# yeeus/GCI

Measured on AMD Instinct MI355X. Metric: aligned Gbases/s through filter+depth pipeline (CHM13, 40x HiFi), higher is better.
Workload: dtype int32

## Files before the change

### gci_amd/csrc/api_ctx.hip

```cpp
#include "gci_ctx.hpp"
#include <stdlib.h>
#include <vector>

int gci_fail(gci_ctx* c, hipError_t e, const char* what)
{
    if (c) c->err = std::string(what) + ": " + hipGetErrorString(e);
    return GCI_E_HIP;
}

int gci_ensure(gci_ctx* ctx, DevBuf& b, size_t bytes)
{
    if (bytes <= b.cap) return GCI_OK;
    if (b.p) { HIPCHK(hipStreamSynchronize(ctx->stream)); HIPCHK(gci_dfree(b.p)); b.p = nullptr; b.cap = 0; }
    size_t want = bytes + bytes / 4 + 256;
    HIPCHK(gci_dmalloc(ctx->device, &b.p, want));
    b.cap = want;
    return GCI_OK;
}

int gci_upload_small(gci_ctx* ctx, void* d_dst, const void* h_src, size_t bytes)
{
    HIPCHK(hipStreamSynchronize(ctx->stream));
    if (bytes > ctx->h_pinned_cap) {
        if (ctx->h_pinned) HIPCHK(hipHostFree(ctx->h_pinned));
// ... 18 lines not shown
    ctx->device = device;
    { const char* fd = getenv("GCI_FORCE_DENSE"); if (fd && fd[0] == '1') ctx->sparse_max = -1; }
    { const char* m = getenv("GCI_JOIN"); ctx->join_mode = m && m[0] == 'c' ? 1 : m && m[0] == 'p' ? 2 : 0; }
    { const char* g = getenv("GCI_PAGES_GRID"); const long n = g ? atol(g) : 0; ctx->pg_grid_cap = n > 0 && n < (1 << 20) ? (uint32_t)n : 0u; }
    hipError_t e = hipSetDevice(device);
    if (e != hipSuccess) { delete ctx; return GCI_E_HIP; }
    if (!own_stream) { ctx->stream = (hipStream_t)stream; }
    else {
        e = hipStreamCreateWithFlags(&ctx->stream, hipStreamNonBlocking);
        if (e != hipSuccess) { delete ctx; return GCI_E_HIP; }
        ctx->own_stream = true;
    }
    {
        uint32_t lut[TEXT_LUT];
        gci_text_lut_host(lut);
        if (gci_dmalloc(device, &ctx->text_lut.p, sizeof lut) != hipSuccess ||
            hipMemcpy(ctx->text_lut.p, lut, sizeof lut, hipMemcpyHostToDevice) != hipSuccess) {
            gci_ctx_destroy(ctx);
            return GCI_E_HIP;
        }
        ctx->text_lut.cap = sizeof lut;
    }
    *out = ctx;
    return GCI_OK;
}

extern "C" int gci_ctx_destroy(gci_ctx* ctx)
{
    if (!ctx) return GCI_OK;
    (void)hipSetDevice(ctx->device);
    (void)hipStreamSynchronize(ctx->stream);
    DevBuf* bufs[] = {&ctx->d_len, &ctx->d_off, &ctx->d_tile_first, &ctx->tile_cd, &ctx->tile_carry, &ctx->dense_flag, &ctx->dense_list, &ctx->evp_items, &ctx->evp_hist, &ctx->evp_blk, &ctx->d_tile_valid,
                      &ctx->evt_off, &ctx->events, &ctx->blk_a, &ctx->blk_b, &ctx->tile_sum, &ctx->tile_u32,
                      &ctx->tile_u64, &ctx->blk_u64, &ctx->join_table, &ctx->join_last, &ctx->join_hq, &ctx->part_a, &ctx->part_b, &ctx->part_hist, &ctx->part_blk, &ctx->conflict_table, &ctx->win,
                      &ctx->win_tile_first, &ctx->text_lut, &ctx->long_items, &ctx->pg_scan, &ctx->pg_first, &ctx->pg_list, &ctx->route_tab, &ctx->deflate_nruns, &ctx->deflate_runs, &ctx->deflate_tab, &ctx->dgz_tiles, &ctx->build_nruns, &ctx->build_runs, &ctx->join_bucket, &ctx->tail_gaps, &ctx->tail_sums, &ctx->class_sums, &ctx->crc_tabs, &ctx->inflate_sym, &ctx->inflate_nsym, &ctx->inflate_wstatus, &ctx->inflate_lists, &ctx->inflate_prof, &ctx->inflate_next, &ctx->inflate_sym2, &ctx->inflate_lists2,
                      &ctx->bg_tile_cnt, &ctx->bg_tile_off, &ctx->bg_blk, &ctx->bg_wtab, &ctx->bg_blk_bytes, &ctx->bg_blk_off, &ctx->bg_blk2, &ctx->hist_chunk_first,
                      &ctx->cover_rec, &ctx->cover_chunk, &ctx->fate_rec, &ctx->fate_chunk};
    for (DevBuf* b : bufs) if (b->p) (void)gci_dfree(b->p);
    for (DevBuf& b : ctx->paf_pool) if (b.p) (void)gci_dfree(b.p);
    if (ctx->h_pinned) (void)hipHostFree(ctx->h_pinned);
    for (auto* v : {&ctx->prof_live, &ctx->prof_free}) for (auto& e : *v) { (void)hipEventDestroy(e.a); (void)hipEventDestroy(e.b); }
    if (ctx->inflate_stream2) { (void)hipStreamSynchronize(ctx->inflate_stream2); (void)hipStreamDestroy(ctx->inflate_stream2); }
    if (ctx->inflate_ev_in) (void)hipEventDestroy(ctx->inflate_ev_in);
    if (ctx->inflate_ev_out) (void)hipEventDestroy(ctx->inflate_ev_out);
    if (ctx->own_stream) (void)hipStreamDestroy(ctx->stream);
    delete ctx;
    return GCI_OK;
}

extern "C" int gci_sync(gci_ctx* ctx)
{
    if (!ctx) return GCI_E_INVALID;
    HIPCHK(hipStreamSynchronize(ctx->stream));
    return GCI_OK;
}

extern "C" const char* gci_strerror(int s)
{
    switch (s) {
    case GCI_OK: return "ok";
    case GCI_E_INVALID: return "invalid argument";
    case GCI_E_HIP: return "HIP runtime error";
    case GCI_E_NO_NM: return "record without NM tag (reference raises KeyError, GCI.py:163)";
    case GCI_E_ZERO_DIV: return "zero denominator (reference raises ZeroDivisionError, GCI.py:165/292)";
    case GCI_E_BAD_NM_TYPE: return "NM tag is not an integer";
    case GCI_E_NO_END: return "record has no CIGAR: reference_end is None";
    case GCI_E_MALFORMED: return "malformed BAM record";
// ... 138 lines not shown
```

### gci_amd/csrc/gci_ctx.hpp

```cpp
#pragma once
#include <hip/hip_runtime.h>
#include <stdint.h>
#include <stdlib.h>
#include <string.h>
#include <string>
#include <vector>

#include "../../include/gci_hip.h"
#include "gci_common.h"
#include "gci_wave.hpp"

#define TILE GCI_TILE
#define TEXT_LUT 1000
#define BLOCK 256
static_assert(TILE == BLOCK * 16, "a tile is 16 elements per thread");

constexpr int GCI_RUN_MAX = 64;
constexpr uint32_t GCI_RUNS_WALK = 0xFFFFFFFFu;

struct DevBuf {
    void* p = nullptr;
    size_t cap = 0;
};

// ... 5 lines not shown
    int32_t n_contigs = 0;
    std::vector<int64_t> len, off;
    std::vector<int64_t> tile_first;
    int64_t total = 0, n_tiles = 0;
    DevBuf d_len, d_off, d_tile_first;
    DevBuf tile_cd;
    DevBuf tile_carry;
    DevBuf evt_off;
    DevBuf d_tile_valid;
    DevBuf dense_flag;
    DevBuf dense_list;
    int32_t sparse_max = 62;
    bool join_dirty = false;
    int join_mode = 0;
    uint32_t k1_parity = 0;
    int cd_state = 0;
    int counted_flank = 0;
    bool count_deferred = false;
    DevBuf evp_items, evp_hist, evp_blk;
    DevBuf events;
    DevBuf blk_a, blk_b;
    DevBuf tile_sum;
    DevBuf tile_u32, tile_u64, blk_u64;
    uint32_t build_max_n = 0;
    int build_flank = 0;
    bool build_pending = false, build_text = false;
    bool build_runs_wanted = false;
    DevBuf build_nruns, build_runs;
    const void* build_runs_track = nullptr;
    bool build_runs_armed = false;
    DevBuf join_table, join_last, join_hq;
    DevBuf join_bucket;
    DevBuf part_a, part_b, part_hist, part_blk;
    DevBuf route_tab;
    DevBuf deflate_nruns, deflate_runs;
    DevBuf deflate_tab;
    bool deflate_tab_ready = false;
    DevBuf dgz_tiles;
    uint32_t dgz_members = 0;
    const void* dgz_key = nullptr;
    bool deflate_from_build = false;
    uint32_t deflate_members = 0;
    const void* deflate_key_depth = nullptr;
    const void* deflate_key_elem = nullptr;
    DevBuf conflict_table;
    uint64_t conflict_slots = 0;
    uint32_t conflict_parity = 0;
    DevBuf text_lut;
    DevBuf long_items;
    DevBuf pg_scan, pg_first;
    uint32_t pg_n_rec = 0, pg_page_bytes = 0, pg_n_pages = 0;
    uint32_t pg_cus = 0;
    uint32_t pg_per_cu = 0, pg_per_cu_page_bytes = 0;
    uint32_t pg_lean_per_cu = 0, pg_lean_page_bytes = 0;
    uint32_t pg_grid_cap = 0;
    DevBuf pg_list;
    uint32_t pg_parity = 0;
    uint64_t pg_blob_off = 0;
    uint64_t pg_blob_bytes = 0;
    std::vector<DevBuf> paf_pool;
    DevBuf crc_tabs;
    bool crc_tabs_ready = false;
    uint32_t inflate_last_n = 0;
    DevBuf inflate_sym, inflate_nsym, inflate_wstatus, inflate_lists, inflate_prof, inflate_next;
    DevBuf inflate_sym2, inflate_lists2;
    int inflate_streams = 1;
// ... 377 lines not shown
```

### gci_amd/csrc/k_join.hip

```cpp
#include "gci_ctx.hpp"
#include <stdlib.h>

struct JoinFiles {
    gci_join_file f[GCI_MAX_JOIN_FILES];
    int n;
};

#define SLOT_EMPTY 0xFFFFFFFFFFFFFFFFull

__device__ __forceinline__ const uint8_t* name_ptr(const gci_join_file& f, uint32_t idx)
{
    return f.d_name_base + f.d_name_off[idx] + f.name_delta;
}

__device__ __forceinline__ bool same_name(const JoinFiles& F, int fa, uint32_t ia, const gci_rec& a,
                                          unsigned long long owner)
{
    const int fb = (int)(owner >> 32);
    const uint32_t ib = (uint32_t)owner;
    const gci_rec& b = F.f[fb].d_recs[ib];
    if (a.name_hash != b.name_hash || a.name_len != b.name_len) return false;
    const uint8_t* pa = name_ptr(F.f[fa], ia);
    const uint8_t* pb = name_ptr(F.f[fb], ib);
    for (uint32_t i = 0; i < a.name_len; i++) if (pa[i] != pb[i]) return false;
// ... 175 lines not shown
    atomicMin(status, (unsigned long long)(unsigned)(-GCI_E_CAPACITY));
}

__device__ __forceinline__ int part_file_of(const PartFiles& P, int n, uint32_t chunk)
{
    int f = 0;
    while (f + 1 < n && chunk >= P.chunk_first[f + 1]) f++;
    return f;
}

__device__ __forceinline__ const uint8_t* entry_name(const JoinFiles& F, const PartEntry& e)
{
    return F.f[(e.meta >> PART_CONTIG_BITS) & 15u].d_name_base + (((uint64_t)e.name_off16 << 4) | (uint64_t)(e.key >> 60));
}

__device__ __forceinline__ void store_entry(PartEntry* __restrict__ dst, const PartEntry& e)
{
    int4* d = reinterpret_cast<int4*>(dst);
    d[0] = make_int4((int)(uint32_t)e.key, (int)(uint32_t)(e.key >> 32), (int)e.idx, (int)e.meta);
    d[1] = make_int4(e.start, e.end, e.qlen, (int)e.name_off16);
}

__device__ __forceinline__ PartEntry load_entry(const PartEntry* __restrict__ src)
{
    const int4* s = reinterpret_cast<const int4*>(src);
    const int4 a = s[0], b = s[1];
    PartEntry e;
    e.key = (unsigned long long)(uint32_t)a.x | ((unsigned long long)(uint32_t)a.y << 32);
    e.idx = (uint32_t)a.z; e.meta = (uint32_t)a.w;
    e.start = b.x; e.end = b.y; e.qlen = b.z; e.name_off16 = (uint32_t)b.w;
    return e;
}

__global__ __launch_bounds__(BLOCK) void k_part1_hist(JoinFiles F, PartFiles P, int shift, uint32_t n_bins, uint32_t n_chunks,
                                                      uint32_t* __restrict__ hist, uint32_t* __restrict__ reset_n_out,
                                                      unsigned long long* __restrict__ status)
{
    __shared__ uint32_t h[256];
    const uint32_t t = threadIdx.x, chunk = blockIdx.x;
    if (chunk == 0 && t == 0) *reset_n_out = 0;
    h[t] = 0;
    __syncthreads();
    const int f = part_file_of(P, F.n, chunk);
    const uint32_t i0 = (chunk - P.chunk_first[f]) * PART_CHUNK, n = F.f[f].n_recs;
    const gci_rec* __restrict__ recs = F.f[f].d_recs;
#pragma unroll 4
    for (int k = 0; k < PART_CHUNK / BLOCK; k++) {
        const uint32_t i = i0 + k * BLOCK + t;
        if (i < n) {
            const gci_rec r = recs[i];
            if (part_takes(r)) atomicAdd(&h[(uint32_t)((r.name_hash & PART_KEY_MASK) >> shift) & (n_bins - 1)], 1u);
            else if (r.flags & GCI_REC_PASS) part_refuse(status);
        }
    }
    __syncthreads();
    if (t < n_bins) hist[(size_t)t * n_chunks + chunk] = h[t];
}

#define SC_TILE 1024
#define SC_PER (SC_TILE / BLOCK)
struct ScatterLds {
    int4 stage[SC_TILE * 2];
    uint32_t tcnt[256], toff[256], gofs[256], cnt[256], base[256];
    uint32_t wtot[BLOCK / 64], total;
    uint8_t sbin[SC_TILE];
};

__device__ __forceinline__ void scatter_tile(ScatterLds& L, const PartEntry (&e)[SC_PER], const int (&d)[SC_PER], uint32_t n_bins,
                                             PartEntry* __restrict__ out, int t)
{
    const int lane = t & 63, wave = t >> 6;
    uint32_t r[SC_PER];
#pragma unroll
    for (int k = 0; k < SC_PER; k++) r[k] = d[k] >= 0 ? atomicAdd(&L.tcnt[d[k]], 1u) : 0u;
    __syncthreads();
    const uint32_t c = (uint32_t)t < n_bins ? L.tcnt[t] : 0u;
    const uint32_t inc = wave_inclusive<uint32_t>(c, lane);
    if (lane == 63) L.wtot[wave] = inc;
    __syncthreads();
    uint32_t pre = inc - c, all = 0;
#pragma unroll
    for (int w = 0; w < BLOCK / 64; w++) { if (w < wave) pre += L.wtot[w]; all += L.wtot[w]; }
    L.toff[t] = pre;
    L.gofs[t] = L.base[t] + L.cnt[t] - pre;
    if (t == 0) L.total = all;
    __syncthreads();
#pragma unroll
    for (int k = 0; k < SC_PER; k++) {
        if (d[k] >= 0) {
            const uint32_t p = L.toff[d[k]] + r[k];
            L.stage[2 * p] = make_int4((int)(uint32_t)e[k].key, (int)(uint32_t)(e[k].key >> 32), (int)e[k].idx, (int)e[k].meta);
            L.stage[2 * p + 1] = make_int4(e[k].start, e[k].end, e[k].qlen, (int)e[k].name_off16);
            L.sbin[p] = (uint8_t)d[k];
        }
    }
    __syncthreads();
    const uint32_t total = L.total;
    for (uint32_t q = t; q < 2 * total; q += BLOCK) {
        const uint32_t p = q >> 1;
        const uint32_t bin = L.sbin[p];
        reinterpret_cast<int4*>(out + (L.gofs[bin] + p))[q & 1] = L.stage[q];
    }
    L.cnt[t] += c;
    L.tcnt[t] = 0;
    __syncthreads();
}

__global__ __launch_bounds__(BLOCK) void k_part1_scatter(JoinFiles F, PartFiles P, int shift, uint32_t n_bins, uint32_t n_chunks,
                                                         const uint32_t* __restrict__ off, PartEntry* __restrict__ out,
                                                         unsigned long long* __restrict__ status)
{
    __shared__ ScatterLds L;
    const uint32_t t = threadIdx.x, chunk = blockIdx.x;
    L.cnt[t] = 0; L.tcnt[t] = 0;
    L.base[t] = t < n_bins ? off[(size_t)t * n_chunks + chunk] : 0u;
    __syncthreads();
    const int f = part_file_of(P, F.n, chunk);
    const uint32_t i0 = (chunk - P.chunk_first[f]) * PART_CHUNK, n = F.f[f].n_recs;
    const gci_rec* __restrict__ recs = F.f[f].d_recs;
    const uint64_t* __restrict__ noff = F.f[f].d_name_off;
    const uint64_t delta = F.f[f].name_delta;
    for (uint32_t tile = 0; tile < PART_CHUNK && i0 + tile < n; tile += SC_TILE) {
        PartEntry e[SC_PER];
        int d[SC_PER];
#pragma unroll
        for (int k = 0; k < SC_PER; k++) {
            const uint32_t i = i0 + tile + k * BLOCK + t;
            d[k] = -1;
            e[k].key = 0; e[k].idx = 0; e[k].meta = 0; e[k].start = e[k].end = e[k].qlen = 0; e[k].name_off16 = 0;
            if (i < n) {
                const gci_rec r = recs[i];
                if (part_takes(r)) {
                    const uint64_t at = noff[i] + delta;
                    if (at >> 36) part_refuse(status);
                    e[k].key = (r.name_hash & PART_KEY_MASK) | ((unsigned long long)r.name_len << 48) | ((unsigned long long)(at & 15ull) << 60);
                    e[k].idx = i;
                    e[k].meta = (uint32_t)r.contig | ((uint32_t)f << PART_CONTIG_BITS) | ((r.flags & GCI_REC_HQ) ? 1u << 30 : 0u) |
                                ((r.flags & GCI_REC_NAME16) ? 1u << 31 : 0u);
                    e[k].start = r.start; e[k].end = r.end; e[k].qlen = r.qlen;
                    e[k].name_off16 = (uint32_t)(at >> 4);
                    d[k] = (int)((uint32_t)((e[k].key & PART_KEY_MASK) >> shift) & (n_bins - 1));
                }
            }
        }
        scatter_tile(L, e, d, n_bins, out, (int)t);
    }
}

__global__ __launch_bounds__(BLOCK) void k_part_mid(const uint32_t* __restrict__ off1, uint32_t n_bins, uint32_t n_chunks,
                                                    uint32_t* __restrict__ seg)
{
    __shared__ uint32_t s[257], c[257];
    const uint32_t t = threadIdx.x;
    if (t <= n_bins) s[t] = off1[(size_t)t * n_chunks];
    if (t == 0 && n_bins == 256) s[256] = off1[(size_t)256 * n_chunks];
    __syncthreads();
    if (t == 0) {
        uint32_t acc = 0;
        for (uint32_t d = 0; d < n_bins; d++) { c[d] = acc; acc += (s[d + 1] - s[d] + PART_CHUNK - 1) / PART_CHUNK; }
        c[n_bins] = acc;
    }
    __syncthreads();
    if (t <= n_bins) { seg[t] = s[t]; seg[n_bins + 1 + t] = c[t]; }
    if (t == 0 && n_bins == 256) { seg[256] = s[256]; seg[513] = c[256]; }
}

__device__ __forceinline__ bool part2_chunk(const uint32_t* sS, const uint32_t* sC, uint32_t n_seg, uint32_t w, uint32_t& j,
                                            uint32_t& k, uint32_t& a, uint32_t& b, uint32_t& nch)
{
    if (w >= sC[n_seg]) return false;
    uint32_t lo = 0, hi = n_seg;
    while (hi - lo > 1) { const uint32_t mid = (lo + hi) >> 1; if (sC[mid] <= w) lo = mid; else hi = mid; }
    j = lo; k = w - sC[j]; nch = sC[j + 1] - sC[j];
    a = sS[j] + k * PART_CHUNK;
    b = min(sS[j + 1], a + PART_CHUNK);
    return true;
}

__global__ __launch_bounds__(BLOCK) void k_part2_hist(const PartEntry* __restrict__ in, const uint32_t* __restrict__ seg,
                                                      uint32_t n_seg, int shift, uint32_t n_bins, uint32_t* __restrict__ hist)
{
    __shared__ uint32_t sS[257], sC[257], h[256];
    const uint32_t t = threadIdx.x, w = blockIdx.x;
    for (uint32_t i = t; i <= n_seg; i += BLOCK) { sS[i] = seg[i]; sC[i] = seg[n_seg + 1 + i]; }
    h[t] = 0;
    __syncthreads();
    uint32_t j, k, a, b, nch;
    if (!part2_chunk(sS, sC, n_seg, w, j, k, a, b, nch)) {
        if (t < n_bins) hist[(size_t)w * n_bins + t] = 0;
        return;
    }
    for (uint32_t i = a + t; i < b; i += BLOCK)
        atomicAdd(&h[(uint32_t)((in[i].key & PART_KEY_MASK) >> shift) & (n_bins - 1)], 1u);
    __syncthreads();
    if (t < n_bins) hist[(size_t)sC[j] * n_bins + (size_t)t * nch + k] = h[t];
}

__global__ __launch_bounds__(BLOCK) void k_part2_scatter(const PartEntry* __restrict__ in, const uint32_t* __restrict__ seg,
                                                         uint32_t n_seg, int shift, uint32_t n_bins,
                                                         const uint32_t* __restrict__ off, PartEntry* __restrict__ out)
{
    __shared__ ScatterLds L;
    __shared__ uint32_t sS[257], sC[257];
    const uint32_t t = threadIdx.x, w = blockIdx.x;
    for (uint32_t i = t; i <= n_seg; i += BLOCK) { sS[i] = seg[i]; sC[i] = seg[n_seg + 1 + i]; }
    L.cnt[t] = 0; L.tcnt[t] = 0;
    __syncthreads();
    uint32_t j, k, a, b, nch;
    if (!part2_chunk(sS, sC, n_seg, w, j, k, a, b, nch)) return;
    L.base[t] = t < n_bins ? off[(size_t)sC[j] * n_bins + (size_t)t * nch + k] : 0u;
    __syncthreads();
    for (uint32_t tile = a; tile < b; tile += SC_TILE) {
        PartEntry e[SC_PER];
        int d[SC_PER];
#pragma unroll
        for (int q = 0; q < SC_PER; q++) {
            const uint32_t i = tile + q * BLOCK + t;
            d[q] = -1;
            e[q].key = 0; e[q].idx = 0; e[q].meta = 0; e[q].start = e[q].end = e[q].qlen = 0; e[q].name_off16 = 0;
            if (i < b) {
                e[q] = load_entry(in + i);
                d[q] = (int)((uint32_t)((e[q].key & PART_KEY_MASK) >> shift) & (n_bins - 1));
            }
        }
        scatter_tile(L, e, d, n_bins, out, (int)t);
    }
// ... 20 lines not shown
                uint32_t x = __builtin_amdgcn_alignbyte(a[k + 1], a[k], sa) ^ __builtin_amdgcn_alignbyte(b[k + 1], b[k], sb);
                const uint32_t left = len - 4u * w;
                if (left < 4u) x &= (1u << (8u * left)) - 1u;
                diff |= x;
            }
        }
    }
    return diff == 0;
}

__device__ __forceinline__ bool names_equal16(const uint8_t* __restrict__ pa, const uint8_t* __restrict__ pb, uint32_t len)
{
    const uint32_t s = (uint32_t)((uintptr_t)pa & 15u);
    const uint4* __restrict__ qa = reinterpret_cast<const uint4*>(pa - s);
    const uint4* __restrict__ qb = reinterpret_cast<const uint4*>(pb - s);
    const uint32_t end = s + len;
    const uint4 z = make_uint4(0, 0, 0, 0);
    const uint4 a0 = qa[0], b0 = qb[0];
    const uint4 a1 = end > 16 ? qa[1] : z, b1 = end > 16 ? qb[1] : z;
    const uint4 a2 = end > 32 ? qa[2] : z, b2 = end > 32 ? qb[2] : z;
    uint32_t d = (s ? 0u : a0.x ^ b0.x) | (a0.y ^ b0.y) | (a0.z ^ b0.z) | (a0.w ^ b0.w);
    d |= (a1.x ^ b1.x) | (a1.y ^ b1.y) | (a1.z ^ b1.z) | (a1.w ^ b1.w);
    d |= (a2.x ^ b2.x) | (a2.y ^ b2.y) | (a2.z ^ b2.z) | (a2.w ^ b2.w);
    return d == 0;
}

struct PartJoinArgs {
    const PartEntry* in; const uint32_t* seg; const uint32_t* off2;
    uint32_t n_seg, n_bins2, slots, slot_shift;
};

template <bool CLAIM>
__device__ __forceinline__ uint32_t part_probe(unsigned long long* meta, uint32_t S, uint32_t slot_shift, const PartEntry& e, uint32_t i,
                                               const PartEntry* __restrict__ in, const JoinFiles& F, bool exact, uint16_t* used,
                                               uint32_t* s_used)
{
    const unsigned long long tag = e.key & 0xFFFFFFFFFFull;
    uint32_t slot = (uint32_t)((e.key & PART_KEY_MASK) >> slot_shift) & (S - 1);
    for (uint32_t probes = 0; probes < S; probes++) {
        unsigned long long m = meta[slot];
        if (m == SLOT_EMPTY) {
            if (!CLAIM) return PART_NONE;
            m = atomicCAS(meta + slot, SLOT_EMPTY, (tag << 24) | ((unsigned long long)i << 1));
            if (m == SLOT_EMPTY) {
                used[atomicAdd(s_used, 1u)] = (uint16_t)slot;
                return slot;
            }
        }
        if ((m >> 24) == tag) {
            if (!exact) return slot;
            const uint32_t c = (uint32_t)(m >> 1) & 0x7FFFFFu;
            if (c == i) return slot;
            const PartEntry ce = load_entry(in + c);
            if (((ce.key ^ e.key) & PART_CMP_MASK) == 0 &&
                names_equal(entry_name(F, e), entry_name(F, ce), (uint32_t)(e.key >> 48) & 0xFFFu))
                return slot;
        }
        slot = (slot + 1) & (S - 1);
    }
    return PART_NONE;
}

template <int FN>
__device__ __forceinline__ bool fold_bucket_slot(const JoinFiles& F, const PartEntry* __restrict__ in, uint32_t slot,
                                                 const unsigned long long* last, bool high, double ovlp_percent,
                                                 const int32_t* __restrict__ contig_map, unsigned long long* __restrict__ status,
                                                 gci_ivl& o)
{
    constexpr int NF = FN ? FN : 1;
    const int Fn = FN ? FN : F.n;
    bool have = false, dead = false;
    int32_t contig = -1, s = 0, e = 0;
    const uint32_t cmask = (1u << PART_CONTIG_BITS) - 1u;
    if constexpr (FN != 0) {
        unsigned long long v[NF];
        int4 ra[NF], rb[NF];
        bool comm = true;
#pragma unroll
        for (int f = 0; f < NF; f++) { v[f] = last[(size_t)slot * NF + f]; comm = comm && v[f] != 0; }
#pragma unroll
// ... 84 lines not shown
                const int64_t ovlp = (int64_t)me - (int64_t)ms;
                if (r.w == 0) {
                    const uint32_t idx = in[(uint32_t)(v & 0x7FFFFFull)].idx;
                    atomicMin(status, ((unsigned long long)F.f[f].d_recs[idx].rec_idx << 8) | (unsigned)(-GCI_E_ZERO_DIV));
                    return false;
                }
                if ((double)ovlp / (double)r.w < ovlp_percent) have = false;
                else { s = ms; e = me; }
            } else have = false;
        } else {
            have = true; contig = r_contig; s = r.y; e = r.z;
        }
    }
    if (!have) return false;
    if (contig_map) { contig = contig_map[contig]; if (contig < 0) return false; }
    o.contig = contig; o.start = s; o.end = e; o.pad = 0;
    return true;
}

#ifndef PART_E
#define PART_E 2
#endif
#ifndef JB
#define JB 512
#endif
template <int FN>
__global__ __launch_bounds__(JB) __attribute__((amdgpu_waves_per_eu(4, 4))) void k_join_part(JoinFiles F, PartJoinArgs A, double ovlp_percent,
                                                     const int32_t* __restrict__ contig_map, gci_ivl* __restrict__ sparse,
                                                     uint32_t* __restrict__ bucket_cnt, uint32_t* __restrict__ bucket_lo,
                                                     unsigned long long* __restrict__ status, const CountArgs cnt)
{
    extern __shared__ __attribute__((aligned(16))) unsigned long long sm[];
    __shared__ uint32_t wtot[JB / 64];
    __shared__ uint32_t s_used, s_bad;
    __shared__ int64_t s_len[COUNT_LDS], s_tf[COUNT_LDS];
    const uint32_t S = A.slots;
    const int Fn = FN ? FN : F.n;
    unsigned long long* meta = sm;
    unsigned long long* cname = sm + S;
    unsigned long long* last = sm + 2 * (size_t)S;
    int4* pay = reinterpret_cast<int4*>(sm + 2 * (size_t)S + (size_t)S * Fn);
    uint16_t* used = reinterpret_cast<uint16_t*>(sm + 2 * (size_t)S + 3 * (size_t)S * Fn);
    const int t = threadIdx.x, lane = t & 63, wave = t >> 6;
    const uint32_t j = blockIdx.x / A.n_bins2, d = blockIdx.x % A.n_bins2;
    const uint32_t cj = A.seg[A.n_seg + 1 + j], nch = A.seg[A.n_seg + 2 + j] - cj;
    if (nch == 0) { if (t == 0) bucket_cnt[blockIdx.x] = 0u; return; }
    const uint32_t lo = A.off2[(size_t)cj * A.n_bins2 + (size_t)d * nch], hi = A.off2[(size_t)cj * A.n_bins2 + (size_t)(d + 1) * nch];
    if (t == 0) { bucket_cnt[blockIdx.x] = 0u; bucket_lo[blockIdx.x] = lo; }
    if (lo == hi) return;
    const bool tables_in_lds = cnt.tile_cd && cnt.n_contigs <= COUNT_LDS;
    if (tables_in_lds) for (int c = t; c < cnt.n_contigs; c += JB) { s_len[c] = cnt.len[c]; s_tf[c] = cnt.tile_first[c]; }
    const PartEntry* __restrict__ in = A.in + lo;
    const uint32_t n = hi - lo;
    if (n >> 23) {
        if (t == 0) part_refuse(status);
        return;
    }
    const uint32_t cmask = (1u << PART_CONTIG_BITS) - 1u;
    const bool in_regs = n <= PART_E * JB;
    PartEntry ent[PART_E];
    uint32_t slot_of[PART_E];
#pragma unroll
    for (int k = 0; k < PART_E; k++) {
        slot_of[k] = PART_NONE;
        const uint32_t i = (uint32_t)t + (uint32_t)k * JB;
        if (in_regs && i < n) ent[k] = load_entry(in + i);
        else { ent[k].key = 0; ent[k].idx = 0; ent[k].meta = 0; ent[k].start = ent[k].end = ent[k].qlen = 0; ent[k].name_off16 = 0; }
    }
    auto name_word = [](const PartEntry& e) -> unsigned long long {
        return (unsigned long long)e.name_off16 | ((e.key >> 60) << 32) | (((e.key >> 48) & 0xFFFull) << 36) |
               ((unsigned long long)((e.meta >> PART_CONTIG_BITS) & 15u) << 48) | ((unsigned long long)(e.meta >> 31) << 52);
    };
    auto insert = [&](const PartEntry& e, uint32_t i, bool exact) -> uint32_t {
        const uint32_t slot = part_probe<true>(meta, S, A.slot_shift, e, i, in, F, exact, used, &s_used);
        if (slot == PART_NONE) { part_refuse(status); return slot; }
        if (((uint32_t)(meta[slot] >> 1) & 0x7FFFFFu) == i) cname[slot] = name_word(e);
        const int file = (int)((e.meta >> PART_CONTIG_BITS) & 15u);
        const unsigned long long ord = (((unsigned long long)(e.meta & cmask) << 32) | e.idx) + 1ull;
        atomicMax(last + (size_t)slot * Fn + file, ord);
        if (Fn > 1 && (e.meta >> 30 & 1u)) atomicOr(meta + slot, 1ull);
        return slot;
    };
    auto settle = [&](const PartEntry& e, uint32_t i, uint32_t slot, bool exact) {
        const int file = (int)((e.meta >> PART_CONTIG_BITS) & 15u);
        const unsigned long long ord = (((unsigned long long)(e.meta & cmask) << 32) | e.idx) + 1ull;
        if (last[(size_t)slot * Fn + file] == ord) {
            last[(size_t)slot * Fn + file] = PART_WIN | i;
            pay[(size_t)slot * Fn + file] = make_int4((int)(e.meta & cmask), e.start, e.end, e.qlen);
        }
        if (!exact && ((uint32_t)(meta[slot] >> 1) & 0x7FFFFFu) != i) {
            const unsigned long long cw = cname[slot];
            const uint32_t len = (uint32_t)(e.key >> 48) & 0xFFFu;
            const uint8_t* cn = F.f[(cw >> 48) & 15u].d_name_base + (((cw & 0xFFFFFFFFull) << 4) | ((cw >> 32) & 15ull));
            const uint8_t* mn = entry_name(F, e);
            bool same;
            if (((uint32_t)(cw >> 36) & 0xFFFu) != len) same = false;
            else if ((e.meta >> 31) && ((cw >> 52) & 1ull) && len <= 44u && (((uintptr_t)mn ^ (uintptr_t)cn) & 15u) == 0)
                same = names_equal16(mn, cn, len);
            else same = names_equal(mn, cn, len);
            if (!same) s_bad = 1u;
        }
    };
    bool exact = false;
    for (;;) {
        for (uint32_t s = t; s < S; s += JB) meta[s] = SLOT_EMPTY;
        for (uint32_t s = t; s < S * (uint32_t)Fn; s += JB) last[s] = 0ull;
        if (t == 0) { s_used = 0; s_bad = 0; }
        __syncthreads();
        if (in_regs) {
#pragma unroll
            for (int k = 0; k < PART_E; k++) {
                const uint32_t i = (uint32_t)t + (uint32_t)k * JB;
                if (i < n) slot_of[k] = insert(ent[k], i, exact);
            }
        } else {
            for (uint32_t i = t; i < n; i += JB) insert(load_entry(in + i), i, exact);
        }
        __syncthreads();
        if (in_regs) {
#pragma unroll
            for (int k = 0; k < PART_E; k++) {
                const uint32_t i = (uint32_t)t + (uint32_t)k * JB;
                if (i < n && slot_of[k] != PART_NONE) settle(ent[k], i, slot_of[k], exact);
            }
        } else {
            for (uint32_t i = t; i < n; i += JB) {
                const PartEntry e = load_entry(in + i);
                const uint32_t slot = part_probe<false>(meta, S, A.slot_shift, e, i, in, F, exact, used, &s_used);
                if (slot != PART_NONE) settle(e, i, slot, exact);
            }
        }
        __syncthreads();
        if (exact || !s_bad) break;
        exact = true;
        __syncthreads();
    }
    auto fold_one = [&](const PartEntry& e, uint32_t i, uint32_t slot, gci_ivl& keep) -> bool {
        const int file = (int)((e.meta >> PART_CONTIG_BITS) & 15u);
        if (last[(size_t)slot * Fn + file] != (PART_WIN | i)) return false;
        for (int f = 0; f < file; f++) if (last[(size_t)slot * Fn + f] != 0) return false;
        return fold_from_entry<FN>(F, in, e, file, slot, last, pay, (meta[slot] & 1ull) != 0, ovlp_percent, contig_map, status, keep);
    };
    auto emit = [&](const gci_ivl& keep, uint32_t w) {
        sparse[lo + w] = keep;
        if (cnt.tile_cd) {
            const IvlSpan sp = tables_in_lds ? span_of(keep, cnt.flank, s_len, s_tf, cnt.n_contigs)
                                             : span_of(keep, cnt.flank, cnt.len, cnt.tile_first, cnt.n_contigs);
            if (sp.valid) count_span(sp, cnt.tile_cd);
        }
    };
    if (in_regs) {
        gci_ivl keep[PART_E];
        bool ok[PART_E];
        uint32_t mine = 0;
#pragma unroll
        for (int k = 0; k < PART_E; k++) {
            const uint32_t i = (uint32_t)t + (uint32_t)k * JB;
            ok[k] = i < n && slot_of[k] != PART_NONE && fold_one(ent[k], i, slot_of[k], keep[k]);
            mine += ok[k] ? 1u : 0u;
        }
        const uint32_t inc = wave_inclusive<uint32_t>(mine, lane);
        if (lane == 63) wtot[wave] = inc;
        __syncthreads();
        uint32_t pre = inc - mine, all = 0;
#pragma unroll
        for (int w = 0; w < JB / 64; w++) { if (w < wave) pre += wtot[w]; all += wtot[w]; }
        if (t == 0) bucket_cnt[blockIdx.x] = all;
        uint32_t w = pre;
#pragma unroll
        for (int k = 0; k < PART_E; k++) if (ok[k]) emit(keep[k], w++);
    } else {
        uint32_t run = 0;
        for (uint32_t i0 = 0; i0 < n; i0 += JB) {
            const uint32_t i = i0 + t;
            gci_ivl keep;
            bool ok = false;
            if (i < n) {
                const PartEntry e = load_entry(in + i);
                const uint32_t slot = part_probe<false>(meta, S, A.slot_shift, e, i, in, F, exact, used, &s_used);
                ok = slot != PART_NONE && fold_one(e, i, slot, keep);
            }
            const unsigned long long bal = __ballot(ok);
            if (lane == 0) wtot[wave] = (uint32_t)__builtin_popcountll(bal);
            __syncthreads();
            uint32_t pre = (uint32_t)__builtin_popcountll(bal & ((1ull << lane) - 1ull)), all = 0;
#pragma unroll
            for (int w = 0; w < JB / 64; w++) { if (w < wave) pre += wtot[w]; all += wtot[w]; }
            if (ok) emit(keep, run + pre);
            run += all;
            __syncthreads();
        }
        if (t == 0) bucket_cnt[blockIdx.x] = run;
    }
}

__global__ __launch_bounds__(BLOCK) void k_join_gather(const gci_ivl* __restrict__ sparse, const uint32_t* __restrict__ bucket_cnt,
                                                       const uint32_t* __restrict__ bucket_lo, const uint32_t* __restrict__ off,
                                                       uint32_t n_buckets, gci_ivl* __restrict__ out, uint32_t cap, uint32_t* __restrict__ n_out)
{
    const uint32_t b = blockIdx.x * (BLOCK / 64) + (threadIdx.x >> 6), lane = threadIdx.x & 63;
    if (blockIdx.x == 0 && threadIdx.x == 0) *n_out = off[n_buckets];
    if (b >= n_buckets) return;
    const uint32_t c = bucket_cnt[b];
    if (!c) return;
    const gci_ivl* __restrict__ src = sparse + bucket_lo[b];
    const uint32_t o = off[b];
    for (uint32_t r = lane; r < c; r += 64) if (o + r < cap) out[o + r] = src[r];
}

static int name_join_partitioned(gci_ctx* ctx, const JoinFiles& F, uint64_t total, double ovlp_percent,
                                 const int32_t* d_contig_map, gci_ivl* d_out, uint32_t cap, uint32_t* d_n_out,
                                 uint64_t* d_status, const CountArgs& cnt, bool* done)
{
    *done = false;
    uint32_t S = 1024;
    while (S > 128 && (size_t)S * (16 + 24 * (size_t)F.n) > 65536) S >>= 1;
    uint64_t nb = 256;
    while (nb * S * 5 < total * 8) nb <<= 1;
    if (nb > 65536) return GCI_OK;
    int bits = 0;
    while ((1ull << bits) < nb) bits++;
    const int b1 = (bits + 1) / 2, b2 = bits - b1;
    const uint32_t B1 = 1u << b1, B2 = 1u << b2;
    int s_bits = 0;
    while ((1u << s_bits) < S) s_bits++;
    const int shift1 = 48 - b1, shift2 = 48 - b1 - b2, slot_shift = shift2 - s_bits;
    PartFiles P;
    uint32_t C1 = 0;
    for (int f = 0; f < F.n; f++) { P.chunk_first[f] = C1; C1 += (F.f[f].n_recs + PART_CHUNK - 1) / PART_CHUNK; }
    for (int f = F.n; f <= GCI_MAX_JOIN_FILES; f++) P.chunk_first[f] = C1;
    const uint32_t C2 = (uint32_t)(total / PART_CHUNK) + B1 + 1;
    const size_t n1 = (size_t)B1 * C1, n2 = (size_t)C2 * B2;
    GCI_TRY(gci_ensure(ctx, ctx->part_a, total * sizeof(PartEntry) + 16));
    GCI_TRY(gci_ensure(ctx, ctx->part_b, total * sizeof(PartEntry) + 16));
    GCI_TRY(gci_ensure(ctx, ctx->part_hist, (n1 + 1 + n2 + 1 + 2 * (size_t)B1 + 2) * 4 + 64));
    GCI_TRY(gci_ensure(ctx, ctx->part_blk, ((n1 > n2 ? n1 : n2) / TILE + 2) * 4));
    uint32_t* hist1 = (uint32_t*)ctx->part_hist.p;
    uint32_t* hist2 = hist1 + n1 + 1;
    uint32_t* seg = hist2 + n2 + 1;
    PartEntry* pa = (PartEntry*)ctx->part_a.p;
    PartEntry* pb = (PartEntry*)ctx->part_b.p;
    HIPCHK(hipMemsetAsync(d_status, 0xFF, 8, ctx->stream));
    {
        ProfScope _ps(ctx, GCI_PROF_PARTITION);
        hipLaunchKernelGGL(k_part1_hist, dim3(C1), dim3(BLOCK), 0, ctx->stream, F, P, shift1, B1, C1, hist1, d_n_out,
                           (unsigned long long*)d_status);
        LAUNCHCHK("k_part1_hist");
        int r = device_exclusive_scan<uint32_t, uint32_t>(ctx, hist1, hist1, (uint32_t*)ctx->part_blk.p, (int64_t)n1, true);
        if (r) return r;
        hipLaunchKernelGGL(k_part1_scatter, dim3(C1), dim3(BLOCK), 0, ctx->stream, F, P, shift1, B1, C1, (const uint32_t*)hist1, pa,
                           (unsigned long long*)d_status);
        LAUNCHCHK("k_part1_scatter");
        hipLaunchKernelGGL(k_part_mid, dim3(1), dim3(BLOCK), 0, ctx->stream, (const uint32_t*)hist1, B1, C1, seg);
        LAUNCHCHK("k_part_mid");
        hipLaunchKernelGGL(k_part2_hist, dim3(C2), dim3(BLOCK), 0, ctx->stream, (const PartEntry*)pa, (const uint32_t*)seg, B1,
                           shift2, B2, hist2);
        LAUNCHCHK("k_part2_hist");
        r = device_exclusive_scan<uint32_t, uint32_t>(ctx, hist2, hist2, (uint32_t*)ctx->part_blk.p, (int64_t)n2, true);
        if (r) return r;
        hipLaunchKernelGGL(k_part2_scatter, dim3(C2), dim3(BLOCK), 0, ctx->stream, (const PartEntry*)pa, (const uint32_t*)seg, B1,
                           shift2, B2, (const uint32_t*)hist2, pb);
        LAUNCHCHK("k_part2_scatter");
    }
    {
        ProfScope _ps(ctx, GCI_PROF_JOIN_PART);
        PartJoinArgs A;
        A.in = pb; A.seg = seg; A.off2 = hist2; A.n_seg = B1; A.n_bins2 = B2; A.slots = S; A.slot_shift = (uint32_t)slot_shift;
        const size_t lds = (size_t)S * (16 + 24 * (size_t)F.n) + (size_t)S * 2;
        const dim3 grid(B1 * B2), block(JB);
        const uint32_t NB = B1 * B2;
        GCI_TRY(gci_ensure(ctx, ctx->join_bucket, ((size_t)3 * NB + 2) * 4 + 64));
        uint32_t* bcnt = (uint32_t*)ctx->join_bucket.p;
        uint32_t* blo = bcnt + NB;
        uint32_t* boff = blo + NB;
        gci_ivl* sparse = (gci_ivl*)pa;
        static_assert(sizeof(gci_ivl) <= sizeof(PartEntry), "the sparse intervals fit the partition buffer");
        const void* kfn = F.n == 1 ? (const void*)k_join_part<1> : F.n == 2 ? (const void*)k_join_part<2> : F.n == 3 ? (const void*)k_join_part<3>
                        : F.n == 4 ? (const void*)k_join_part<4> : (const void*)k_join_part<0>;
        HIPCHK(hipFuncSetAttribute(kfn, hipFuncAttributeMaxDynamicSharedMemorySize, (int)lds));
        switch (F.n) {
        case 1: hipLaunchKernelGGL((k_join_part<1>), grid, block, lds, ctx->stream, F, A, ovlp_percent, d_contig_map, sparse, bcnt, blo, (unsigned long long*)d_status, cnt); break;
        case 2: hipLaunchKernelGGL((k_join_part<2>), grid, block, lds, ctx->stream, F, A, ovlp_percent, d_contig_map, sparse, bcnt, blo, (unsigned long long*)d_status, cnt); break;
        case 3: hipLaunchKernelGGL((k_join_part<3>), grid, block, lds, ctx->stream, F, A, ovlp_percent, d_contig_map, sparse, bcnt, blo, (unsigned long long*)d_status, cnt); break;
        case 4: hipLaunchKernelGGL((k_join_part<4>), grid, block, lds, ctx->stream, F, A, ovlp_percent, d_contig_map, sparse, bcnt, blo, (unsigned long long*)d_status, cnt); break;
        default: hipLaunchKernelGGL((k_join_part<0>), grid, block, lds, ctx->stream, F, A, ovlp_percent, d_contig_map, sparse, bcnt, blo, (unsigned long long*)d_status, cnt); break;
        }
        LAUNCHCHK("k_join_part");
        int r2 = device_exclusive_scan<uint32_t, uint32_t>(ctx, bcnt, boff, (uint32_t*)ctx->part_blk.p, (int64_t)NB, true);
        if (r2) return r2;
        hipLaunchKernelGGL(k_join_gather, dim3((NB + BLOCK / 64 - 1) / (BLOCK / 64)), dim3(BLOCK), 0, ctx->stream, (const gci_ivl*)sparse,
                           (const uint32_t*)bcnt, (const uint32_t*)blo, (const uint32_t*)boff, NB, d_out, cap, d_n_out);
        LAUNCHCHK("k_join_gather");
    }
    *done = true;
    return GCI_OK;
}

static int name_join_impl(gci_ctx* ctx, const gci_join_file* h_files, int n_files, double ovlp_percent,
                          const int32_t* d_contig_map, gci_ivl* d_out, uint32_t cap, uint32_t* d_n_out,
                          uint64_t* d_status, const CountArgs& cnt)
{
// ... 246 lines not shown
```

Measured before the change: 25130.

## Precompute second-pass partition bins in scatter and batch record loads

The first-pass scatter now also writes a one-byte second-pass bin index per entry into a new buffer. The second histogram can then read those compact bytes with vectorized 16-byte loads instead of re-reading full 32-byte partition entries. Record loads in both first-pass kernels are batched ahead of use to raise memory-level parallelism. The unused slot-tracking list in the join probe is removed, which saves shared memory and an atomic per insert. The cost is an extra byte-wide scattered write per entry plus one more device buffer.

```diff
diff --git a/gci_amd/csrc/api_ctx.hip b/gci_amd/csrc/api_ctx.hip
--- a/gci_amd/csrc/api_ctx.hip
+++ b/gci_amd/csrc/api_ctx.hip
@@ -74,7 +74,7 @@
     (void)hipStreamSynchronize(ctx->stream);
     DevBuf* bufs[] = {&ctx->d_len, &ctx->d_off, &ctx->d_tile_first, &ctx->tile_cd, &ctx->tile_carry, &ctx->dense_flag, &ctx->dense_list, &ctx->evp_items, &ctx->evp_hist, &ctx->evp_blk, &ctx->d_tile_valid,
                       &ctx->evt_off, &ctx->events, &ctx->blk_a, &ctx->blk_b, &ctx->tile_sum, &ctx->tile_u32,
-                      &ctx->tile_u64, &ctx->blk_u64, &ctx->join_table, &ctx->join_last, &ctx->join_hq, &ctx->part_a, &ctx->part_b, &ctx->part_hist, &ctx->part_blk, &ctx->conflict_table, &ctx->win,
+                      &ctx->tile_u64, &ctx->blk_u64, &ctx->join_table, &ctx->join_last, &ctx->join_hq, &ctx->part_a, &ctx->part_b, &ctx->part_hist, &ctx->part_blk, &ctx->part_next, &ctx->conflict_table, &ctx->win,
                       &ctx->win_tile_first, &ctx->text_lut, &ctx->long_items, &ctx->pg_scan, &ctx->pg_first, &ctx->pg_list, &ctx->route_tab, &ctx->deflate_nruns, &ctx->deflate_runs, &ctx->deflate_tab, &ctx->dgz_tiles, &ctx->build_nruns, &ctx->build_runs, &ctx->join_bucket, &ctx->tail_gaps, &ctx->tail_sums, &ctx->class_sums, &ctx->crc_tabs, &ctx->inflate_sym, &ctx->inflate_nsym, &ctx->inflate_wstatus, &ctx->inflate_lists, &ctx->inflate_prof, &ctx->inflate_next, &ctx->inflate_sym2, &ctx->inflate_lists2,
                       &ctx->bg_tile_cnt, &ctx->bg_tile_off, &ctx->bg_blk, &ctx->bg_wtab, &ctx->bg_blk_bytes, &ctx->bg_blk_off, &ctx->bg_blk2, &ctx->hist_chunk_first,
                       &ctx->cover_rec, &ctx->cover_chunk, &ctx->fate_rec, &ctx->fate_chunk};
diff --git a/gci_amd/csrc/gci_ctx.hpp b/gci_amd/csrc/gci_ctx.hpp
--- a/gci_amd/csrc/gci_ctx.hpp
+++ b/gci_amd/csrc/gci_ctx.hpp
@@ -61,6 +61,7 @@
     DevBuf join_table, join_last, join_hq;
     DevBuf join_bucket;
     DevBuf part_a, part_b, part_hist, part_blk;
+    DevBuf part_next;
     DevBuf route_tab;
     DevBuf deflate_nruns, deflate_runs;
     DevBuf deflate_tab;
diff --git a/gci_amd/csrc/k_join.hip b/gci_amd/csrc/k_join.hip
--- a/gci_amd/csrc/k_join.hip
+++ b/gci_amd/csrc/k_join.hip
@@ -231,6 +231,7 @@
     return e;
 }
 
+#define H1_PER 4
 __global__ __launch_bounds__(BLOCK) void k_part1_hist(JoinFiles F, PartFiles P, int shift, uint32_t n_bins, uint32_t n_chunks,
                                                       uint32_t* __restrict__ hist, uint32_t* __restrict__ reset_n_out,
                                                       unsigned long long* __restrict__ status)
@@ -243,13 +244,18 @@
     const int f = part_file_of(P, F.n, chunk);
     const uint32_t i0 = (chunk - P.chunk_first[f]) * PART_CHUNK, n = F.f[f].n_recs;
     const gci_rec* __restrict__ recs = F.f[f].d_recs;
-#pragma unroll 4
-    for (int k = 0; k < PART_CHUNK / BLOCK; k++) {
-        const uint32_t i = i0 + k * BLOCK + t;
-        if (i < n) {
-            const gci_rec r = recs[i];
-            if (part_takes(r)) atomicAdd(&h[(uint32_t)((r.name_hash & PART_KEY_MASK) >> shift) & (n_bins - 1)], 1u);
-            else if (r.flags & GCI_REC_PASS) part_refuse(status);
+#pragma unroll 1
+    for (int k0 = 0; k0 < PART_CHUNK / BLOCK; k0 += H1_PER) {
+        gci_rec r[H1_PER];
+#pragma unroll
+        for (int k = 0; k < H1_PER; k++) r[k] = recs[min(i0 + (k0 + k) * BLOCK + t, n - 1)];
+        asm volatile("" ::: "memory");
+#pragma unroll
+        for (int k = 0; k < H1_PER; k++) {
+            if (i0 + (k0 + k) * BLOCK + t < n) {
+                if (part_takes(r[k])) atomicAdd(&h[(uint32_t)((r[k].name_hash & PART_KEY_MASK) >> shift) & (n_bins - 1)], 1u);
+                else if (r[k].flags & GCI_REC_PASS) part_refuse(status);
+            }
         }
     }
     __syncthreads();
@@ -266,7 +272,8 @@
 };
 
 __device__ __forceinline__ void scatter_tile(ScatterLds& L, const PartEntry (&e)[SC_PER], const int (&d)[SC_PER], uint32_t n_bins,
-                                             PartEntry* __restrict__ out, int t)
+                                             PartEntry* __restrict__ out, int t, uint8_t* __restrict__ next = nullptr,
+                                             int next_shift = 0, uint32_t next_mask = 0)
 {
     const int lane = t & 63, wave = t >> 6;
     uint32_t r[SC_PER];
@@ -298,7 +305,12 @@
     for (uint32_t q = t; q < 2 * total; q += BLOCK) {
         const uint32_t p = q >> 1;
         const uint32_t bin = L.sbin[p];
-        reinterpret_cast<int4*>(out + (L.gofs[bin] + p))[q & 1] = L.stage[q];
+        const int4 v = L.stage[q];
+        reinterpret_cast<int4*>(out + (L.gofs[bin] + p))[q & 1] = v;
+        if (next && !(q & 1)) {
+            const unsigned long long key = (unsigned long long)(uint32_t)v.x | ((unsigned long long)(uint32_t)v.y << 32);
+            next[L.gofs[bin] + p] = (uint8_t)((uint32_t)((key & PART_KEY_MASK) >> next_shift) & next_mask);
+        }
     }
     L.cnt[t] += c;
     L.tcnt[t] = 0;
@@ -307,6 +319,7 @@
 
 __global__ __launch_bounds__(BLOCK) void k_part1_scatter(JoinFiles F, PartFiles P, int shift, uint32_t n_bins, uint32_t n_chunks,
                                                          const uint32_t* __restrict__ off, PartEntry* __restrict__ out,
+                                                         uint8_t* __restrict__ next, int next_shift, uint32_t next_mask,
                                                          unsigned long long* __restrict__ status)
 {
     __shared__ ScatterLds L;
@@ -322,27 +335,31 @@
     for (uint32_t tile = 0; tile < PART_CHUNK && i0 + tile < n; tile += SC_TILE) {
         PartEntry e[SC_PER];
         int d[SC_PER];
+        gci_rec r[SC_PER];
+        uint64_t no[SC_PER];
+#pragma unroll
+        for (int k = 0; k < SC_PER; k++) r[k] = recs[min(i0 + tile + k * BLOCK + t, n - 1)];
+#pragma unroll
+        for (int k = 0; k < SC_PER; k++) no[k] = noff[min(i0 + tile + k * BLOCK + t, n - 1)];
+        asm volatile("" ::: "memory");
 #pragma unroll
         for (int k = 0; k < SC_PER; k++) {
             const uint32_t i = i0 + tile + k * BLOCK + t;
             d[k] = -1;
             e[k].key = 0; e[k].idx = 0; e[k].meta = 0; e[k].start = e[k].end = e[k].qlen = 0; e[k].name_off16 = 0;
-            if (i < n) {
-                const gci_rec r = recs[i];
-                if (part_takes(r)) {
-                    const uint64_t at = noff[i] + delta;
-                    if (at >> 36) part_refuse(status);
-                    e[k].key = (r.name_hash & PART_KEY_MASK) | ((unsigned long long)r.name_len << 48) | ((unsigned long long)(at & 15ull) << 60);
-                    e[k].idx = i;
-                    e[k].meta = (uint32_t)r.contig | ((uint32_t)f << PART_CONTIG_BITS) | ((r.flags & GCI_REC_HQ) ? 1u << 30 : 0u) |
-                                ((r.flags & GCI_REC_NAME16) ? 1u << 31 : 0u);
-                    e[k].start = r.start; e[k].end = r.end; e[k].qlen = r.qlen;
-                    e[k].name_off16 = (uint32_t)(at >> 4);
-                    d[k] = (int)((uint32_t)((e[k].key & PART_KEY_MASK) >> shift) & (n_bins - 1));
-                }
-            }
-        }
-        scatter_tile(L, e, d, n_bins, out, (int)t);
+            if (i < n && part_takes(r[k])) {
+                const uint64_t at = no[k] + delta;
+                if (at >> 36) part_refuse(status);
+                e[k].key = (r[k].name_hash & PART_KEY_MASK) | ((unsigned long long)r[k].name_len << 48) | ((unsigned long long)(at & 15ull) << 60);
+                e[k].idx = i;
+                e[k].meta = (uint32_t)r[k].contig | ((uint32_t)f << PART_CONTIG_BITS) | ((r[k].flags & GCI_REC_HQ) ? 1u << 30 : 0u) |
+                            ((r[k].flags & GCI_REC_NAME16) ? 1u << 31 : 0u);
+                e[k].start = r[k].start; e[k].end = r[k].end; e[k].qlen = r[k].qlen;
+                e[k].name_off16 = (uint32_t)(at >> 4);
+                d[k] = (int)((uint32_t)((e[k].key & PART_KEY_MASK) >> shift) & (n_bins - 1));
+            }
+        }
+        scatter_tile(L, e, d, n_bins, out, (int)t, next, next_shift, next_mask);
     }
 }
 
@@ -376,8 +393,8 @@
     return true;
 }
 
-__global__ __launch_bounds__(BLOCK) void k_part2_hist(const PartEntry* __restrict__ in, const uint32_t* __restrict__ seg,
-                                                      uint32_t n_seg, int shift, uint32_t n_bins, uint32_t* __restrict__ hist)
+__global__ __launch_bounds__(BLOCK) void k_part2_hist(const uint8_t* __restrict__ bins, const uint32_t* __restrict__ seg,
+                                                      uint32_t n_seg, uint32_t n_bins, uint32_t* __restrict__ hist)
 {
     __shared__ uint32_t sS[257], sC[257], h[256];
     const uint32_t t = threadIdx.x, w = blockIdx.x;
@@ -389,8 +406,15 @@
         if (t < n_bins) hist[(size_t)w * n_bins + t] = 0;
         return;
     }
-    for (uint32_t i = a + t; i < b; i += BLOCK)
-        atomicAdd(&h[(uint32_t)((in[i].key & PART_KEY_MASK) >> shift) & (n_bins - 1)], 1u);
+    const uint32_t a16 = min(b, (a + 15u) & ~15u), b16 = max(a16, b & ~15u);
+    for (uint32_t i = a + t; i < a16; i += BLOCK) atomicAdd(&h[bins[i]], 1u);
+    for (uint32_t i = a16 + 16u * t; i < b16; i += 16u * BLOCK) {
+        const uint4 v = *reinterpret_cast<const uint4*>(bins + i);
+        const uint32_t four[4] = {v.x, v.y, v.z, v.w};
+#pragma unroll
+        for (int q = 0; q < 16; q++) atomicAdd(&h[(four[q >> 2] >> (8 * (q & 3))) & 0xFFu], 1u);
+    }
+    for (uint32_t i = b16 + t; i < b; i += BLOCK) atomicAdd(&h[bins[i]], 1u);
     __syncthreads();
     if (t < n_bins) hist[(size_t)sC[j] * n_bins + (size_t)t * nch + k] = h[t];
 }
@@ -477,8 +501,7 @@
 
 template <bool CLAIM>
 __device__ __forceinline__ uint32_t part_probe(unsigned long long* meta, uint32_t S, uint32_t slot_shift, const PartEntry& e, uint32_t i,
-                                               const PartEntry* __restrict__ in, const JoinFiles& F, bool exact, uint16_t* used,
-                                               uint32_t* s_used)
+                                               const PartEntry* __restrict__ in, const JoinFiles& F, bool exact)
 {
     const unsigned long long tag = e.key & 0xFFFFFFFFFFull;
     uint32_t slot = (uint32_t)((e.key & PART_KEY_MASK) >> slot_shift) & (S - 1);
@@ -487,10 +510,7 @@
         if (m == SLOT_EMPTY) {
             if (!CLAIM) return PART_NONE;
             m = atomicCAS(meta + slot, SLOT_EMPTY, (tag << 24) | ((unsigned long long)i << 1));
-            if (m == SLOT_EMPTY) {
-                used[atomicAdd(s_used, 1u)] = (uint16_t)slot;
-                return slot;
-            }
+            if (m == SLOT_EMPTY) return slot;
         }
         if ((m >> 24) == tag) {
             if (!exact) return slot;
@@ -641,7 +661,7 @@
 {
     extern __shared__ __attribute__((aligned(16))) unsigned long long sm[];
     __shared__ uint32_t wtot[JB / 64];
-    __shared__ uint32_t s_used, s_bad;
+    __shared__ uint32_t s_bad;
     __shared__ int64_t s_len[COUNT_LDS], s_tf[COUNT_LDS];
     const uint32_t S = A.slots;
     const int Fn = FN ? FN : F.n;
@@ -649,7 +669,6 @@
     unsigned long long* cname = sm + S;
     unsigned long long* last = sm + 2 * (size_t)S;
     int4* pay = reinterpret_cast<int4*>(sm + 2 * (size_t)S + (size_t)S * Fn);
-    uint16_t* used = reinterpret_cast<uint16_t*>(sm + 2 * (size_t)S + 3 * (size_t)S * Fn);
     const int t = threadIdx.x, lane = t & 63, wave = t >> 6;
     const uint32_t j = blockIdx.x / A.n_bins2, d = blockIdx.x % A.n_bins2;
     const uint32_t cj = A.seg[A.n_seg + 1 + j], nch = A.seg[A.n_seg + 2 + j] - cj;
@@ -681,7 +700,7 @@
                ((unsigned long long)((e.meta >> PART_CONTIG_BITS) & 15u) << 48) | ((unsigned long long)(e.meta >> 31) << 52);
     };
     auto insert = [&](const PartEntry& e, uint32_t i, bool exact) -> uint32_t {
-        const uint32_t slot = part_probe<true>(meta, S, A.slot_shift, e, i, in, F, exact, used, &s_used);
+        const uint32_t slot = part_probe<true>(meta, S, A.slot_shift, e, i, in, F, exact);
         if (slot == PART_NONE) { part_refuse(status); return slot; }
         if (((uint32_t)(meta[slot] >> 1) & 0x7FFFFFu) == i) cname[slot] = name_word(e);
         const int file = (int)((e.meta >> PART_CONTIG_BITS) & 15u);
@@ -714,7 +733,7 @@
     for (;;) {
         for (uint32_t s = t; s < S; s += JB) meta[s] = SLOT_EMPTY;
         for (uint32_t s = t; s < S * (uint32_t)Fn; s += JB) last[s] = 0ull;
-        if (t == 0) { s_used = 0; s_bad = 0; }
+        if (t == 0) s_bad = 0;
         __syncthreads();
         if (in_regs) {
 #pragma unroll
@@ -735,7 +754,7 @@
         } else {
             for (uint32_t i = t; i < n; i += JB) {
                 const PartEntry e = load_entry(in + i);
-                const uint32_t slot = part_probe<false>(meta, S, A.slot_shift, e, i, in, F, exact, used, &s_used);
+                const uint32_t slot = part_probe<false>(meta, S, A.slot_shift, e, i, in, F, exact);
                 if (slot != PART_NONE) settle(e, i, slot, exact);
             }
         }
@@ -786,7 +805,7 @@
             bool ok = false;
             if (i < n) {
                 const PartEntry e = load_entry(in + i);
-                const uint32_t slot = part_probe<false>(meta, S, A.slot_shift, e, i, in, F, exact, used, &s_used);
+                const uint32_t slot = part_probe<false>(meta, S, A.slot_shift, e, i, in, F, exact);
                 ok = slot != PART_NONE && fold_one(e, i, slot, keep);
             }
             const unsigned long long bal = __ballot(ok);
@@ -842,6 +861,7 @@
     const size_t n1 = (size_t)B1 * C1, n2 = (size_t)C2 * B2;
     GCI_TRY(gci_ensure(ctx, ctx->part_a, total * sizeof(PartEntry) + 16));
     GCI_TRY(gci_ensure(ctx, ctx->part_b, total * sizeof(PartEntry) + 16));
+    GCI_TRY(gci_ensure(ctx, ctx->part_next, total + 16));
     GCI_TRY(gci_ensure(ctx, ctx->part_hist, (n1 + 1 + n2 + 1 + 2 * (size_t)B1 + 2) * 4 + 64));
     GCI_TRY(gci_ensure(ctx, ctx->part_blk, ((n1 > n2 ? n1 : n2) / TILE + 2) * 4));
     uint32_t* hist1 = (uint32_t*)ctx->part_hist.p;
@@ -849,6 +869,7 @@
     uint32_t* seg = hist2 + n2 + 1;
     PartEntry* pa = (PartEntry*)ctx->part_a.p;
     PartEntry* pb = (PartEntry*)ctx->part_b.p;
+    uint8_t* bins2 = (uint8_t*)ctx->part_next.p;
     HIPCHK(hipMemsetAsync(d_status, 0xFF, 8, ctx->stream));
     {
         ProfScope _ps(ctx, GCI_PROF_PARTITION);
@@ -858,12 +879,12 @@
         int r = device_exclusive_scan<uint32_t, uint32_t>(ctx, hist1, hist1, (uint32_t*)ctx->part_blk.p, (int64_t)n1, true);
         if (r) return r;
         hipLaunchKernelGGL(k_part1_scatter, dim3(C1), dim3(BLOCK), 0, ctx->stream, F, P, shift1, B1, C1, (const uint32_t*)hist1, pa,
-                           (unsigned long long*)d_status);
+                           bins2, shift2, B2 - 1, (unsigned long long*)d_status);
         LAUNCHCHK("k_part1_scatter");
         hipLaunchKernelGGL(k_part_mid, dim3(1), dim3(BLOCK), 0, ctx->stream, (const uint32_t*)hist1, B1, C1, seg);
         LAUNCHCHK("k_part_mid");
-        hipLaunchKernelGGL(k_part2_hist, dim3(C2), dim3(BLOCK), 0, ctx->stream, (const PartEntry*)pa, (const uint32_t*)seg, B1,
-                           shift2, B2, hist2);
+        hipLaunchKernelGGL(k_part2_hist, dim3(C2), dim3(BLOCK), 0, ctx->stream, (const uint8_t*)bins2, (const uint32_t*)seg, B1, B2,
+                           hist2);
         LAUNCHCHK("k_part2_hist");
         r = device_exclusive_scan<uint32_t, uint32_t>(ctx, hist2, hist2, (uint32_t*)ctx->part_blk.p, (int64_t)n2, true);
         if (r) return r;
@@ -875,7 +896,7 @@
         ProfScope _ps(ctx, GCI_PROF_JOIN_PART);
         PartJoinArgs A;
         A.in = pb; A.seg = seg; A.off2 = hist2; A.n_seg = B1; A.n_bins2 = B2; A.slots = S; A.slot_shift = (uint32_t)slot_shift;
-        const size_t lds = (size_t)S * (16 + 24 * (size_t)F.n) + (size_t)S * 2;
+        const size_t lds = (size_t)S * (16 + 24 * (size_t)F.n);
         const dim3 grid(B1 * B2), block(JB);
         const uint32_t NB = B1 * B2;
         GCI_TRY(gci_ensure(ctx, ctx->join_bucket, ((size_t)3 * NB + 2) * 4 + 64));
```

Result: no change. 25270 (median of 2 runs) (+0.6%).
